# ayotoasset/AdditiveCausalExpansion

Measured on AMD Instinct MI355X. Metric: log-marg-lik+grad evals/sec at n=16384,d=20; Cholesky GF/s vs MFMA peak, higher is better.
Workload: dtype f64; 1 GPU; C2: n=16384, d=20, Matern32, ns basis B=10, fp64; one para_update (kernel assembly + SPD inverse/log-det + all P gradients + RMSE/evidence + Nadam step) per step; n=16384, p=20, B=10, kernel=Matern32, parallelism=single

## Files before the change

### additivecausalexpansion_amd/__init__.py

```python
from ._lib import AceError, Context, default_context, lib
from .native import (
    DMat, Adam_cpp, Nadam_cpp, Nesterov_cpp, coef_contract, grad_Matern_cpp, grad_SE_cpp,
    invkernel_cpp, kernmat_Matern32_cpp, kernmat_Matern32_symmetric_cpp, kernmat_SE_cpp,
    kernmat_SE_symmetric_cpp, mu_solution_cpp, ncs_basis, ncs_basis_deriv, norm_clip_cpp,
    normalize_test, normalize_train, pred_cpp, pred_marginal_cpp, robust_levels, stats_cpp,
    zero_pattern_order)
from .model import (
    BatchModel, DeviceModel, KernelClass_Matern32_R6, KernelClass_SE_R6, comm_unique_id, optAdam,
    optNadam, optNesterov, set_optimizer)
from .r6 import R6KernelMatern32, R6KernelSE
from .train import (
    AceFit, ace_train, ace_train_batch, coef_posterior, linear_spline, ns_spline, predict_ace,
    response_surface, robust_treatment, set_basis, set_initial_parameters, square_spline)
```

### additivecausalexpansion_amd/_lib.py

```python
from __future__ import annotations

import ctypes
import os
import threading

import numpy as np

_HERE = os.path.dirname(os.path.abspath(__file__))
LIB_PATH = os.environ.get("ACE_LIB_PATH") or os.path.join(_HERE, "libace_hip.so")

ACE_KERNEL_SE = 0
ACE_KERNEL_MATERN32 = 1
KIND = {"SE": ACE_KERNEL_SE, "Matern32": ACE_KERNEL_MATERN32}

_D = ctypes.POINTER(ctypes.c_double)
_I64 = ctypes.c_int64
_I32 = ctypes.POINTER(ctypes.c_int32)
_vp = ctypes.c_void_p

SIGNATURES = {
    "ace_abi_version": (ctypes.c_int, []),
    "ace_create": (ctypes.c_int, [ctypes.c_int, ctypes.POINTER(_vp)]),
    "ace_destroy": (None, [_vp]),
    "ace_last_error": (ctypes.c_char_p, [_vp]),
# ... 37 lines not shown
                                             ctypes.c_double, _vp, _vp, _vp, ctypes.c_double,
                                             ctypes.c_double, ctypes.c_double, ctypes.c_int, _D,
                                             _D, _D, _D]),
    "ace_nesterov": (ctypes.c_int, [_I64, ctypes.c_double, ctypes.c_double, _D, _D, _D]),
    "ace_nadam": (ctypes.c_int, [_I64, ctypes.c_double, ctypes.c_double, ctypes.c_double,
                                 ctypes.c_double, ctypes.c_double, _D, _D, _D, _D]),
    "ace_adam": (ctypes.c_int, [_I64, ctypes.c_double, ctypes.c_double, ctypes.c_double,
                                ctypes.c_double, ctypes.c_double, _D, _D, _D, _D]),
    "ace_norm_clip": (None, [ctypes.c_int, _I64, _D, ctypes.c_double]),
    "ace_ncs_basis": (ctypes.c_int, [_I64, _D, _I64, _D, _D, ctypes.POINTER(_I64)]),
    "ace_ncs_basis_deriv": (ctypes.c_int, [_I64, _D, _I64, _D, _D, ctypes.POINTER(_I64)]),
    "ace_normalize_train": (ctypes.c_int, [_I64, ctypes.c_int, ctypes.c_int, _D, _D, _D, _D]),
    "ace_normalize_test": (ctypes.c_int, [_I64, ctypes.c_int, ctypes.c_int, _D, _D, _D, _I64]),
    "ace_zero_pattern_order": (ctypes.c_int, [_I64, ctypes.c_int, _D, ctypes.POINTER(_I64),
                                              ctypes.POINTER(ctypes.c_uint32), _I32]),
    "ace_model_create": (ctypes.c_int, [_vp, ctypes.c_int, _I64, ctypes.c_int, ctypes.c_int,
                                        ctypes.POINTER(_vp)]),
    "ace_model_destroy": (None, [_vp]),
    "ace_model_set_data": (ctypes.c_int, [_vp, _D, _D, _D, ctypes.c_double]),
    "ace_model_para_update": (ctypes.c_int, [_vp, ctypes.c_int, _D, _D, _D, _D]),
    "ace_model_train_stats": (ctypes.c_int, [_vp, _D, _D]),
    "ace_model_get_inverse": (ctypes.c_int, [_vp, _D]),
    "ace_model_apply_inverse": (ctypes.c_int, [_vp, _I64, _D, _D]),
    "ace_model_predict": (ctypes.c_int, [_vp, _D, _I64, _D, _D, ctypes.c_double, ctypes.c_double,
                                         _D, _D, _D]),
    "ace_model_predict_marginal": (ctypes.c_int, [_vp, _D, _I64, _D, _D, _D, ctypes.c_double,
                                                  ctypes.c_double, ctypes.c_int, _D, _D, _D,
                                                  _D]),
    "ace_model_predict_marginal_groups": (ctypes.c_int, [_vp, _D, _I64, _D, _D, ctypes.c_double,
                                                         ctypes.c_double, ctypes.c_int, _I32, _D,
# ... 144 lines not shown
```

### additivecausalexpansion_amd/csrc/ace_api.cpp

```cpp
#include <hip/hip_runtime.h>
#include <hip/hip_ext.h>

#include <algorithm>
#include <chrono>
#include <cmath>
#include <cstdio>
#include <cstring>
#include <limits>
#include <string>
#include <thread>
#include <vector>

#include "../../include/ace_hip.h"

#include "ace_common.h"
#include "ace_internal.h"
#include "ace_model.h"

using namespace ace;

std::string g_create_err;

namespace {
double sync_timeout_s() {
// ... 430 lines not shown
  return v;
}
static bool asm_fill_on() {
  static const bool v = env_int("ACE_ASM_FILL", 1) != 0;
  return v;
}

struct AsmFill {
  int kind, PM, B, ZS, slots;
  PairSide ps;
  int64_t npad, naug;
  TabView tv;
  double sig;
  double *A;
  int *queue;
};

static hipError_t asm_fill(void *arg, hipStream_t st) {
  const AsmFill *f = (const AsmFill *)arg;
  return launch_assembly_persist(f->kind, f->PM, f->ps, f->npad, f->B, f->ZS, f->tv, f->sig, f->A,
                                 f->naug, st, f->queue, 0, f->slots);
}

void assemble_and_sweep(ace_ctx *ctx, SweepWork &w, const Shape &s, const PairSide &ps,
                        const TabView &tv, double sig, const double *y, int64_t n,
                        const SweepTiming *tmg, hipEvent_t *ev_asm) {
  hipStream_t st = ctx->stream;
  const int steps = (int)(w.npad / NB);
  SweepSync sy = w.sync(ctx);
  const int R = asm_persist_reserve();
  const bool persist = R > 0 && sy.side && sy.nev >= 5 * steps + 6 && pairs_use_mm(s.PM, false) &&
                       mm_lds_ok(s.PM, s.B, s.kind, false);
  ck(ctx, launch_aug_init(w.A.d(), w.naug, w.npad, n, y, st, 1, 0, w.flag.i(), 1,
                          persist ? w.aq.i() : nullptr, persist ? 2 + 64 : 0),
     "aug init");
  if (ev_asm) ck(ctx, hipEventRecord(ev_asm[0], st), "event");
  ck(ctx, launch_assembly(0, s.kind, s.PM, ps, ps, w.npad, s.B, s.ZS, tv, sig, w.A.d(), w.naug,
                          nullptr, st, nullptr, 0, 1, 1),
     "assembly (first panel)");
  if (sy.side && sy.nev >= 2 * steps + 1) {
    ck(ctx, hipEventRecord(sy.ev[2 * steps], st), "event");
    sy.ready_recorded = true;
  }
  AsmFill fill;
  if (persist && sy.ready_recorded) {
    ck(ctx, launch_assembly_persist(s.kind, s.PM, ps, w.npad, s.B, s.ZS, tv, sig, w.A.d(), w.naug,
                                    st, w.aq.i(), R),
       "assembly (persistent)");
    const int tail = asm_tail_mode();
    if (tail == 0) {
      sy.tail_after = sy.ev[5 * steps + 5];
      ck(ctx, hipEventRecord(sy.tail_after, st), "event");
    }
    sy.tail_split = tail == 2;
    const int per = asm_fill_on() ? assembly_persist_per_cu(s.kind, s.PM, s.B) : 0;
    if (per > 0) {
      fill = AsmFill{s.kind, s.PM, s.B, s.ZS, 32 * R * per, ps, w.npad, w.naug, tv, sig, w.A.d(), w.aq.i()};
      sy.fill = asm_fill;
      sy.fill_arg = &fill;
    }
  } else {
    ck(ctx, launch_assembly(0, s.kind, s.PM, ps, ps, w.npad, s.B, s.ZS, tv, sig, w.A.d(), w.naug,
                            nullptr, st, nullptr, 0, 1, 2),
       "assembly");
  }
  if (ev_asm) ck(ctx, hipEventRecord(ev_asm[1], st), "event");
  ck(ctx, run_sweep(w.bufs(), st, &sy, tmg), "sweep");
}

void build_grad_tiles(ace_ctx *ctx, int64_t n, DBuf &tiles, int64_t *ntiles, int64_t *ndiag,
                      const uint32_t *mask) {
  *ntiles = grad_ntiles(n);
// ... 52 lines not shown
    tv.ldn = m->npad;
  }
  const int ts = m->tset;
  SweepTiming tmg;
  const size_t nset = m->ev_upd.size() / 2;
  tmg.ev = m->ev_upd.data() + ts * nset;
  tmg.nev = (int)nset;
  tmg.used = &m->upd_used[ts];
  tmg.flops = m->upd_flops.data() + ts * (nset / 2);
  assemble_and_sweep(ctx, w, s, ps, tv, sig, m->y.d(), m->n, timed ? &tmg : nullptr,
                     timed ? m->ev_asm + 2 * ts : nullptr);
  ck(ctx, launch_alpha_from_aug(w.A.d(), w.naug, w.npad, m->n, theta_dev ? 0.0 : theta[1], use_mu,
                                m->alpha.d(), m->scal.d(), st, theta_dev ? theta_dev + 1 : nullptr),
     "alpha");
  if (timed) ck(ctx, hipEventRecord(m->ev_grad[2 * ts], st), "event");
  ck(ctx, launch_grad(s.kind, s.PM, ps, s.B, s.ZS, tv, w.A.d(), w.naug, -1.0, m->alpha.d(),
                      nullptr, m->gpart.d(), st, reinterpret_cast<const Tile *>(m->gtiles.p),
                      m->ngdiag >= 0 ? m->ntiles : 0, 1, m->ngdiag),
     "grad");
  if (timed) ck(ctx, hipEventRecord(m->ev_grad[2 * ts + 1], st), "event");
  const int ldg = grad_part_cols(s.PM, s.B);
  ck(ctx, launch_tile_sums(m->gpart.d(), m->ntiles, ldg, m->gwork.d(), m->gsum.d(), st),
     "tile sums");
  ck(ctx, launch_final_sums(m->y.d(), m->scal.d() + 4, m->alpha.d(), nullptr, sig, m->n,
                            w.piv.d(), w.npad, m->sums.d(), st, tv.sig, w.flag.i()),
     "final sums");
}

void model_collect_timing(ace_model *m, int ts) {
  const int nupd = m->upd_used[ts];
  const size_t nset = m->ev_upd.size() / 2;
  const hipEvent_t *ev = m->ev_upd.data() + ts * nset;
  const double *fl = m->upd_flops.data() + ts * (nset / 2);
  float ms = 0.f;
  ck(m->ctx, hipEventElapsedTime(&ms, m->ev_asm[2 * ts], m->ev_asm[2 * ts + 1]), "elapsed");
  m->t_ms[1] += ms;
  m->t_launch[1] += 1;
  ck(m->ctx, hipEventElapsedTime(&ms, m->ev_grad[2 * ts], m->ev_grad[2 * ts + 1]), "elapsed");
  m->t_ms[2] += ms;
  m->t_launch[2] += 1;
  for (int j = 0; j + 1 < nupd; j += 2) {
// ... 139 lines not shown
    alloc(ctx, m->gpart, (size_t)(m->ntiles * ldg) * sizeof(double), "alloc gpart");
    alloc(ctx, m->gwork, (size_t)tile_sums_work(ldg) * sizeof(double), "alloc tile sums");
    alloc(ctx, m->res, (size_t)(ldg + 8 + 16) * sizeof(double), "alloc results");
    m->gsum.p = m->res.d();
    m->sums.p = m->res.d() + ldg;
    m->scal.p = m->res.d() + ldg + 8;
    ck(ctx, hipMemsetAsync(m->sw.A.p, 0, m->sw.A.bytes, ctx->stream), "memset A");
    const int steps = (int)(m->npad / NB);
    m->ev_upd.assign((size_t)(4 * steps), nullptr);
    m->upd_flops.assign((size_t)(2 * steps), 0.0);
    for (auto &e : m->ev_upd) ck(ctx, hipEventCreateWithFlags(&e, ACE_TIMING_EVENT_FLAGS), "event");
    for (int j = 0; j < 4; ++j) {
      ck(ctx, hipEventCreateWithFlags(&m->ev_asm[j], ACE_TIMING_EVENT_FLAGS), "event");
      ck(ctx, hipEventCreateWithFlags(&m->ev_grad[j], ACE_TIMING_EVENT_FLAGS), "event");
    }
    sync(ctx);
  } catch (const Fail &f) {
    ace_model_destroy(m);
    return f.code;
  }
  *out = m;
  return ACE_OK;
}

void ace_model_destroy(ace_model *m) {
  if (!m) return;
  (void)hipSetDevice(m->ctx->device);
  if (m->shard) shard_destroy(m->shard);
  for (auto &e : m->ev_upd)
    if (e) (void)hipEventDestroy(e);
  for (int j = 0; j < 4; ++j) {
    if (m->ev_asm[j]) (void)hipEventDestroy(m->ev_asm[j]);
    if (m->ev_grad[j]) (void)hipEventDestroy(m->ev_grad[j]);
  }
  delete m;
}

int ace_model_set_data(ace_model *m, const double *y, const double *X, const double *Z,
                       double std_y) {
  if (!m) return ACE_ERR_ARG;
  ace_ctx *ctx = m->ctx;
  ACE_TRY
  ck(ctx, hipSetDevice(ctx->device), "hipSetDevice");
  arg(ctx, y && (m->s.p == 0 || X) && (m->s.B == 1 || Z), "null argument");
  if (m->shard) {
    shard_set_data(m->shard, y, X, Z);
    m->std_y = std_y;
    m->has_data = true;
    return ACE_OK;
  }
  const Shape &s = m->s;
  const int64_t n = m->n;
  const int zs = s.B - 1, mode = zskip_mode(n);
  m->perm.clear();
  m->has_zmask = false;
  std::vector<double> Xp, Zp, yp((size_t)m->npad, 0.0);
  std::copy(y, y + n, yp.begin());
  if (mode > 0 && zs >= 1 && zs <= 32 && pairs_use_mm(s.PM, false) &&
      mm_lds_ok(s.PM, s.B, s.kind, false) && mm_lds_ok(s.PM, s.B, s.kind, true)) {
    const uint32_t all = zs >= 32 ? 0xffffffffu : ((uint32_t)1 << zs) - 1;
    std::vector<uint32_t> bm((size_t)(m->npad / AT), all);
    std::vector<int64_t> perm((size_t)n);
    int32_t has = 0;
    arg(ctx, ace_zero_pattern_order(n, zs, Z, perm.data(), bm.data(), &has) == ACE_OK,
        "zero-pattern order");
    bool ident = true;
    for (int64_t k = 0; k < n && ident; ++k) ident = perm[(size_t)k] == k;
    if (mode == 2 && !ident) {
      Xp.resize((size_t)(n * s.p));
      Zp.resize((size_t)(n * zs));
// ... 8 lines not shown
    } else if (!ident) {
      for (int64_t k = 0; k < n / AT; ++k) {
        uint32_t w = 0;
        for (int b = 0; b < zs; ++b)
          for (int64_t j = AT * k; j < AT * (k + 1); ++j)
            if (Z[j + b * n] != 0.0) w |= (uint32_t)1 << b;
        bm[(size_t)k] = w;
      }
    }
    bool any = false;
    for (uint32_t w : bm) any = any || w != all;
    if (any) {
      alloc(ctx, m->zmask, bm.size() * sizeof(uint32_t), "alloc slice masks");
      upload_bytes(ctx, m->zmask.p, bm.data(), bm.size() * sizeof(uint32_t), "upload slice masks");
      m->has_zmask = true;
    }
    int64_t nt = 0;
    build_grad_tiles(ctx, n, m->gtiles, &nt, &m->ngdiag,
                     (any && !m->perm.empty()) ? bm.data() : nullptr);
    arg(ctx, nt == m->ntiles, "gradient tile list changed size");
  }
  upload_side(ctx, m->side, m->s, X, Z, m->n, m->npad);
  upload_bytes(ctx, m->y.p, yp.data(), yp.size() * sizeof(double), "upload y");
  m->std_y = std_y;
  sync(ctx);
  m->has_data = true;
  return ACE_OK;
  ACE_CATCH
}

// ... 303 lines not shown
```

### additivecausalexpansion_amd/csrc/ace_host.cpp

```cpp
#include <algorithm>
#include <cmath>
#include <vector>

#include "../../include/ace_hip.h"

namespace {

bool all_finite(int64_t P, const double *g) {
  for (int64_t j = 0; j < P; ++j)
    if (!std::isfinite(g[j])) return false;
  return true;
}

}

extern "C" {

int ace_nesterov(int64_t P, double learn_rate, double momentum, double *nu, const double *grad,
                 double *para) {
  const bool ok = all_finite(P, grad);
  for (int64_t j = 0; j < P; ++j) {
    nu[j] = momentum * nu[j] + learn_rate * grad[j];
    para[j] = para[j] + nu[j];
  }
// ... 242 lines not shown
  const bool mask = ZS <= 32 && blockmask != nullptr;
  if (has_mask) *has_mask = mask ? 1 : 0;
  if (!mask) return ACE_OK;
  const uint32_t all = ZS >= 32 ? 0xffffffffu : ((uint32_t)1 << ZS) - 1;
  const int64_t nblk = (n + 63) / 64;
  for (int64_t k = 0; k < nblk; ++k) {
    uint32_t m = 0;
    if (64 * (k + 1) > n) m = all;
    else
      for (int64_t j = 64 * k; j < 64 * (k + 1); ++j) m |= (uint32_t)pat[(size_t)perm[j] * W];
    blockmask[k] = m;
  }
  return ACE_OK;
}

int ace_coef_contract(int64_t nx, int B, int64_t nz, const double *mean, const double *cov,
                      const double *W, double offset, double scale, double shift, double noise,
                      double *map, double *ci, double *var) {
  if (nx < 1 || nz < 1 || B < 1 || !mean || !cov || !W || !map || !ci || !var) return ACE_ERR_ARG;
  const int64_t N = nx * nz;
  std::vector<double> wj((size_t)B);
  for (int64_t j = 0; j < nz; ++j) {
    for (int b = 0; b < B; ++b) wj[(size_t)b] = W[j + nz * b];
    for (int64_t c = 0; c < nx; ++c) {
      double a = 0.0, q = 0.0;
      for (int b = 0; b < B; ++b) a += wj[(size_t)b] * mean[c + nx * b];
      for (int b2 = 0; b2 < B; ++b2) {
        double t = 0.0;
        for (int b = 0; b < B; ++b) t += wj[(size_t)b] * cov[c + nx * (b + (int64_t)B * b2)];
        q += t * wj[(size_t)b2];
// ... 15 lines not shown
```

### additivecausalexpansion_amd/csrc/ace_internal.h

```cpp
#pragma once
#include <functional>
#include <vector>
#include <hip/hip_runtime.h>
#include <stdint.h>
#include <stdlib.h>

namespace ace {

inline int env_int(const char *name, int dflt) {
  const char *e = getenv(name);
  return e ? atoi(e) : dflt;
}
inline bool env_set(const char *name) { return getenv(name) != nullptr; }

#ifndef ACE_NB
#define ACE_NB 256
#endif
constexpr int NB = ACE_NB;
constexpr int SUB = 64;
constexpr int UT = 128;
constexpr int AUG = 128;
constexpr int AT = 64;
constexpr int PMAX = 64;
constexpr int BMAX = 32;
// ... 30 lines not shown
hipError_t launch_assembly(int mode, int kind, int PM, PairSide rows,
                           PairSide cols, int64_t npad, int B, int ZS,
                           TabView tab, double sig, double *out, int64_t ld,
                           double *cube, hipStream_t st, const Tile *tiles = nullptr,
                           int64_t ntiles = 0, int G = 1, int part = 0, int b0 = 0,
                           int b1 = -1);
hipError_t launch_kdiag(int kind, PairSide S, int ZS, TabView tab, int b0, int b1, double *out,
                        hipStream_t st);

hipError_t launch_assembly_mm(int kind, int PM, PairSide S, int64_t npad, int B, int ZS,
                              TabView tab, double sig, double *out, int64_t ld,
                              double *kcopy, hipStream_t st, const Tile *tiles,
                              int64_t ntiles, int G, int part = 0);
hipError_t launch_assembly_persist(int kind, int PM, PairSide S, int64_t npad, int B, int ZS,
                                   TabView tab, double sig, double *out, int64_t ld,
                                   hipStream_t st, int *queue, int reserve, int fill = 0);
int assembly_persist_per_cu(int kind, int PM, int B);
bool pairs_use_mm(int PM, bool grad);
bool mm_lds_ok(int PM, int B, int kind, bool grad);
bool cross_mm_lds_ok(int PM, int B, int kind);
hipError_t launch_cross_mm(int kind, int PM, PairSide R, PairSide C, int B, int ZS, TabView tab,
                           int b0, int b1, double *out, int64_t ld, hipStream_t st);
hipError_t launch_cross_slices_mm(int kind, int PM, PairSide R, PairSide C, int B, int ZS,
                                  TabView tab, double *out, int64_t ld, hipStream_t st);
int group_sums_parts(int64_t n);
hipError_t launch_group_sums(int kind, int PM, PairSide S, int B, int ZS, TabView tab, int b0,
                             int b1, const int *label, int G, double *part, double *R,
                             hipStream_t st);
hipError_t launch_grad_mm(int kind, int PM, PairSide S, int B, int ZS, TabView tab,
                          const double *A, int64_t ld, double sA, const double *alpha,
                          double *gpart, hipStream_t st, const Tile *tiles, int64_t ntiles, int G,
                          int64_t ndiag);

__host__ __device__ constexpr int grad_part_cols(int PM, int B) { return B * (PM + 1) + 1; }
hipError_t launch_grad(int kind, int PM, PairSide side, int B, int ZS,
                       TabView tab, const double *A, int64_t ld, double sA,
                       const double *alpha, const double *cube, double *gpart, hipStream_t st,
                       const Tile *tiles = nullptr, int64_t ntiles = 0, int G = 1,
                       int64_t ndiag = -1);
int64_t grad_ntiles(int64_t n);
int grad_order_block();
hipError_t launch_tile_sums(const double *part, int64_t ntiles, int ncols, double *work,
                            double *out, hipStream_t st);
int64_t tile_sums_work(int ncols);

constexpr int64_t SW_DOUBLES = 2 * (int64_t)SUB * SUB + 3 * (int64_t)NB * SUB;
struct SweepBufs {
  double *A;
  int64_t ld;
  int64_t npad;
  double *P[8];
  double *W[8];
  int Z = 2;
  double *SW;
// ... 181 lines not shown
```

### additivecausalexpansion_amd/csrc/ace_model.h

```cpp
#pragma once
#include <functional>

#include "ace_common.h"
#include "ace_internal.h"

struct SweepWork {
  DBuf A, Ps[8], Ws[8], SW, S0, S1, piv, flag, order, xtiles, gorder, htiles;
  int Z = 2;
  DBuf gtiles;
  DBuf aq;
  DBuf bq;
  int breserve = 0;
  int64_t bq_npad = -1;
  int bq_Z = 0;
  DBuf gpart, gwork, gsum;
  DBuf norms;
  int64_t ngtiles = 0, ngdiag = -2;
  std::vector<int64_t> xoff, hoff;
  int64_t glen = 0;
  std::vector<hipEvent_t> ev;
  int64_t n = 0, npad = 0, naug = 0, norder = 0;
  SweepWork() = default;
  SweepWork(const SweepWork &) = delete;
  ~SweepWork() {
    for (auto &e : ev) (void)hipEventDestroy(e);
// ... 1 lines not shown
  void ensure(ace_ctx *ctx, int64_t n_) {
    n = n_;
    npad = round_up(n, NB);
    naug = npad + AUG;
    alloc(ctx, A, (size_t)(naug * naug) * sizeof(double), "alloc A");
    for (int j = 0; j < 2; ++j) {
      alloc(ctx, Ps[j], (size_t)(naug * NB) * sizeof(double), "alloc panel");
      alloc(ctx, Ws[j], (size_t)(naug * NB) * sizeof(double), "alloc panel");
    }
    alloc(ctx, SW, (size_t)SW_DOUBLES * sizeof(double), "alloc SW");
    alloc(ctx, S0, (size_t)(SUB * NB) * sizeof(double), "alloc S");
    alloc(ctx, S1, (size_t)(SUB * NB) * sizeof(double), "alloc S");
    alloc(ctx, piv, (size_t)npad * sizeof(double), "alloc piv");
    alloc(ctx, flag, 16, "alloc flag");
    alloc(ctx, aq, (2 + 64) * sizeof(int), "alloc assembly queue");
    norder = 0;
    if (const int S = update_order_block(); S > 0) {
      const std::vector<Tile> t = xcd_update_order(own_tiles(naug / UT, UT, 1, 0), S);
      alloc(ctx, order, t.size() * sizeof(Tile), "alloc tile order");
      upload_bytes(ctx, order.p, t.data(), t.size() * sizeof(Tile), "upload tile order");
      norder = (int64_t)t.size();
    }
    const int steps = (int)(npad / NB);
    glen = 0;
    hoff.clear();
    if (pair_steps() && steps >= 2) {
      Z = sweep_group_n(naug);
      for (int j = 2; j < 2 * Z; ++j) {
        alloc(ctx, Ps[j], (size_t)(naug * NB) * sizeof(double), "alloc panel");
        alloc(ctx, Ws[j], (size_t)(naug * NB) * sizeof(double), "alloc panel");
// ... 83 lines not shown
  tv.ldn = np;
  return tv;
}

struct ace_model {
  ace_ctx *ctx = nullptr;
  Shape s{};
  int64_t n = 0, npad = 0, naug = 0, ntiles = 0, ntr = 0;
  double std_y = 1.0;
  bool has_data = false;
  bool has_inverse = false;
  SideBufs side;
  std::vector<int64_t> perm;
  DBuf zmask;
  bool has_zmask = false;
  PairSide train_side() const {
    PairSide ps = side.view(n);
    if (has_zmask) ps.mask = static_cast<const uint32_t *>(zmask.p);
    return ps;
  }
  DBuf y, tab, alpha, gpart, gwork;
  DBuf res;
  DView gsum, sums, scal;
  DBuf norms;
  DBuf gtiles;
  int64_t ngdiag = -1;
  PinnedBuf hio;
  SweepWork sw;
  SweepWork sw2;
  bool prof = false;
  hipEvent_t ev_asm[4] = {}, ev_grad[4] = {};
  std::vector<hipEvent_t> ev_upd;
  std::vector<double> upd_flops;
  int upd_used[2] = {0, 0};
  int tset = 0, pend = -1;
  double t_ms[6] = {0, 0, 0, 0, 0, 0};
  int64_t t_launch[6] = {0, 0, 0, 0, 0, 0};
  double t_work[6] = {0, 0, 0, 0, 0, 0};
  ShardModel *shard = nullptr;
};


void assemble_and_sweep(ace_ctx *ctx, SweepWork &w, const Shape &s, const PairSide &ps,
                        const TabView &tv, double sig, const double *y, int64_t n,
                        const SweepTiming *tmg, hipEvent_t *ev_asm);
void build_grad_tiles(ace_ctx *ctx, int64_t n, DBuf &tiles, int64_t *ntiles, int64_t *ndiag,
// ... 20 lines not shown
```

### additivecausalexpansion_amd/csrc/ace_pairs.hip

```cpp
#include <algorithm>
#include <cstdlib>

#include "ace_internal.h"

namespace ace {

#define SQRT3 1.7320508075688772

__device__ __forceinline__ double sgn(double x) {
  return (double)((0.0 < x) - (x < 0.0));
}

template <int KIND, bool CROSS>
__device__ __forceinline__ double kval(int b, double r2, double lam, double zlo,
                                       double zhi, double lzlo, double lzhi) {
  if (KIND == 0) {
    if (b == 0) return exp(lam - r2);
    if (zlo == 0.0 || zhi == 0.0) return 0.0;
    return (sgn(zlo) * sgn(zhi)) * exp(((lam - r2) + lzlo) + lzhi);
  } else {
    const double t = sqrt(r2);
    const double e = (1.0 + SQRT3 * t) * exp(lam - SQRT3 * t);
    if (b == 0) return e;
    if (zlo == 0.0) return 0.0;
// ... 618 lines not shown
    hipLaunchKernelGGL((k_grad2<PM, 1>), grid, blk, 0, st, S, B, ZS, tab, A, ld, sA, alpha,
                       gpart, ldg, tiles, G);
  }
#undef ACE_G
  return hipGetLastError();
}

int grad_order_block() {
  static const int v = std::max(0, env_int("ACE_GRAD_ORDER", 4));
  return v;
}

hipError_t launch_grad(int kind, int PM, PairSide S, int B, int ZS, TabView tab,
                       const double *A, int64_t ld, double sA, const double *alpha,
                       const double *cube, double *gpart, hipStream_t st,
                       const Tile *tiles, int64_t ntiles, int G, int64_t ndiag) {
  const bool valu_ok = PM <= 48;
  if ((!cube || !valu_ok) && (pairs_use_mm(PM, true) || !valu_ok) && mm_lds_ok(PM, B, kind, true))
    return launch_grad_mm(kind, PM, S, B, ZS, tab, A, ld, sA, alpha, gpart, st, tiles, ntiles,
                          G, ndiag);
  if (!valu_ok) return hipErrorInvalidValue;
  switch (PM) {
#define ACE_CASE(P) \
  case P:           \
    return grad_pm<P>(kind, S, B, ZS, tab, A, ld, sA, alpha, cube, gpart, st, tiles, ntiles, G);
    ACE_CASE(4) ACE_CASE(8) ACE_CASE(12) ACE_CASE(16) ACE_CASE(20) ACE_CASE(24)
    ACE_CASE(32) ACE_CASE(48)
#undef ACE_CASE
    default: return hipErrorInvalidValue;
  }
}

}
```

### additivecausalexpansion_amd/csrc/ace_pairs_mm.hip

```cpp
#include <map>
#include <mutex>
#include <tuple>
#include <type_traits>

#include "ace_internal.h"
#include "ace_wgtime.h"

namespace ace {

typedef double d4 __attribute__((ext_vector_type(4)));

#ifndef ACE_MM_PG
#define ACE_MM_PG 2
#endif
#ifndef ACE_MM_GRAD_WPE
#define ACE_MM_GRAD_WPE 4
#endif
#ifndef ACE_MM_QG
#define ACE_MM_QG 4
#endif
#ifndef ACE_MM_QG2
#define ACE_MM_QG2 1
#endif
#ifndef ACE_GRAD_TAIL4
// ... 366 lines not shown
    s = fma(v * v, w[i], s);
  }
  norms[e] = s;
}

hipError_t launch_slice_norms(const double *X, int PM, int64_t np, int B, int NS,
                              const double *wk, const double *wlast, double *norms,
                              hipStream_t st) {
  const int64_t tot = (int64_t)NS * np;
  if (tot == 0) return hipSuccess;
  hipLaunchKernelGGL(k_slice_norms, dim3((unsigned)((tot + 255) / 256)), dim3(256), 0, st, X, PM,
                     np, B, NS, wk, wlast, norms);
  return hipGetLastError();
}

static int asm_first_cols(int nt) {
  const int jb = sweep_group_n((int64_t)nt * AT + AUG) * NB / AT;
  return jb < nt ? jb : nt;
}

constexpr int ASM_NT = 256;
template <int PM, int KIND, bool LOWER = false>
__device__ __forceinline__ void asm_mm_tile(double *lds, PairSide S, int B, int ZS, const TabView &tab,
                                            double sg, double *__restrict__ out, int64_t ld,
                                            double *__restrict__ kcopy, int64_t I, int64_t J,
                                            int G) {
  if (G > 1) {
    const int64_t coff = lcol(J * AT, G) - J * AT;
    out += coff * ld;
    if (kcopy) kcopy += coff * ld;
  }
// ... 226 lines not shown
    cross_slice_pairs<PM, KIND>(kf, XJ, W, Nr, Nc, Zc, LZc, E, xr, tab, b, zr, lzr, rl, lr, lk);
  }
  if (!rok) return;
#pragma unroll
  for (int cb = 0; cb < 4; ++cb)
#pragma unroll
    for (int v = 0; v < 4; ++v) {
      const int64_t c = C0 + 16 * cb + lk + 4 * v;
      if (c < C.n) out[r + c * ld] = kf[cb][v];
    }
}

template <int PM, int KIND>
__global__ __launch_bounds__(ASM_NT, PM <= 24 ? 4 : PM <= 32 ? 3 : 2) void k_asm_mm_q(
    PairSide S, int B, int ZS, TabView tab, double sig, double *__restrict__ out, int64_t ld,
    int *__restrict__ queue, int64_t nblk, int JB, int reserve) {
  extern __shared__ __attribute__((aligned(16))) double lds[];
  __shared__ int next;
  if (reserve > 0) {
    if (threadIdx.x == 0) {
      const unsigned hw = __builtin_amdgcn_s_getreg((31 << 11) | 4);
      const unsigned xcc = __builtin_amdgcn_s_getreg((31 << 11) | 20) & 7;
      const unsigned se = (hw >> 13) & 3;
      const int key = (int)((hw >> 8) & 0xff) + 1;
      int mine = 0;
      for (int r = 0; r < reserve && !mine; ++r) {
        const int old = atomicCAS(queue + 2 + 2 * (4 * xcc + se) + r, 0, key);
        mine = old == 0 || old == key;
      }
      next = mine ? (atomicAdd(queue + 1, 1) < (int)gridDim.x * reserve / 4) : 0;
    }
    __syncthreads();
    if (next) return;
    __syncthreads();
  }
  const double sg = tab.sig ? *tab.sig : sig;
  for (;;) {
    if (threadIdx.x == 0) next = atomicAdd(queue, 1);
    __syncthreads();
    const int64_t idx = next;
    __syncthreads();
    if (idx >= nblk) break;
    int64_t I, J;
    tile_of(nullptr, idx, I, J);
    asm_mm_tile<PM, KIND, true>(lds, S, B, ZS, tab, sg, out, ld, nullptr, I + JB + 1, J + JB, 1);
  }
}

__device__ __forceinline__ double rcp_nr_mm(double f) {
  const double q = __builtin_amdgcn_rcp(f);
  const double e = fma(-f, q, 1.0);
  return fma(q, e, q);
}

template <int CTRL>
__device__ __forceinline__ double dpp64(double v) {
  const unsigned long long u = __double_as_longlong(v);
  const int lo = __builtin_amdgcn_mov_dpp((int)(unsigned)u, CTRL, 0xf, 0xf, false);
  const int hi = __builtin_amdgcn_mov_dpp((int)(unsigned)(u >> 32), CTRL, 0xf, 0xf, false);
  return __longlong_as_double((long long)(((unsigned long long)(unsigned)hi << 32) | (unsigned)lo));
// ... 413 lines not shown
static hipError_t grad_mm_launch_ps(PairSide S, int B, int ZS, TabView tab, const double *A,
                                    int64_t ld, double sA, const double *alpha, double *gpart,
                                    hipStream_t st, const Tile *tiles, int64_t nblk, int G,
                                    size_t lds, int64_t t0) {
  constexpr int CB = grad_cb(PM, KIND);
  constexpr int NT = 64 * 4 * (4 / CB);
  if (nblk == 0) return hipSuccess;
  return launch_lds(k_grad_mm<PM, KIND, CB, PS, DG>, dim3((unsigned)nblk), dim3(NT), lds, st, S, B,
                    ZS, tab, A, ld, sA, alpha, gpart, grad_part_cols(PM, B), tiles, G, t0);
}

template <int PM, int KIND, bool PS>
static hipError_t grad_mm_launch_dg(PairSide S, int B, int ZS, TabView tab, const double *A,
                                    int64_t ld, double sA, const double *alpha, double *gpart,
                                    hipStream_t st, const Tile *tiles, int64_t nslot,
                                    int64_t ndiag, int G, size_t lds) {
  if (tiles && ndiag < 0)
    return grad_mm_launch_ps<PM, KIND, PS, true>(S, B, ZS, tab, A, ld, sA, alpha, gpart, st, tiles,
                                                 nslot, G, lds, 0);
  const int64_t nd = tiles ? ndiag : (S.n + AT - 1) / AT;
  hipError_t e = grad_mm_launch_ps<PM, KIND, PS, false>(S, B, ZS, tab, A, ld, sA, alpha, gpart, st,
                                                        tiles, nslot - nd, G, lds, nd);
  if (e != hipSuccess) return e;
  return grad_mm_launch_ps<PM, KIND, PS, true>(S, B, ZS, tab, A, ld, sA, alpha, gpart, st, tiles,
                                               nd, G, lds, 0);
}

template <int PM, int KIND>
static hipError_t grad_mm_launch(PairSide S, int B, int ZS, TabView tab, const double *A,
                                 int64_t ld, double sA, const double *alpha, double *gpart,
                                 hipStream_t st, const Tile *tiles, int64_t nslot, int64_t ndiag,
                                 int G) {
  constexpr int CB = grad_cb(PM, KIND);
  constexpr int NT = 64 * 4 * (4 / CB);
  const MmLayout o = mm_layout(PM, B, KIND, true, NT / 64);
  const size_t lds = (size_t)o.total * sizeof(double);
  return o.red_slices == B
             ? grad_mm_launch_dg<PM, KIND, true>(S, B, ZS, tab, A, ld, sA, alpha, gpart, st, tiles,
                                                 nslot, ndiag, G, lds)
             : grad_mm_launch_dg<PM, KIND, false>(S, B, ZS, tab, A, ld, sA, alpha, gpart, st,
                                                  tiles, nslot, ndiag, G, lds);
}

bool mm_lds_ok(int PM, int B, int kind, bool grad) {
  const int nwave = grad ? 4 * (4 / grad_cb(PM, kind)) : 4;
  return (int64_t)mm_layout(PM, B, kind == 0 ? 0 : 1, grad, nwave).total *
             (int64_t)sizeof(double) <=
         160 * 1024;
}

hipError_t launch_grad_mm(int kind, int PM, PairSide S, int B, int ZS, TabView tab,
                          const double *A, int64_t ld, double sA, const double *alpha,
                          double *gpart, hipStream_t st, const Tile *tiles, int64_t ntiles, int G,
                          int64_t ndiag) {
  return with_pm(PM, [&](auto pm) {
    const int64_t nt = (S.n + AT - 1) / AT;
    const int64_t nslot = tiles ? ntiles : nt * (nt + 1) / 2;
    if (nslot == 0) return hipSuccess;
    return with_kind(kind, [&](auto kd) {
      return grad_mm_launch<decltype(pm)::value, decltype(kd)::value>(
          S, B, ZS, tab, A, ld, sA, alpha, gpart, st, tiles, nslot, ndiag, G);
    });
  });
}

template <int PM, int KIND>
static hipError_t asm_mm_launch(PairSide S, int64_t npad, int B, int ZS, TabView tab, double sig,
                                double *out, int64_t ld, double *kcopy, hipStream_t st,
                                const Tile *tiles, int64_t ntiles, int G, int part) {
  const int64_t nt = npad / AT, JB = asm_first_cols((int)nt);
  if (tiles) part = 0;
  const int64_t nblk = tiles ? ntiles
                       : part == 1 ? JB * nt - JB * (JB - 1) / 2
                       : part == 2 ? (nt - JB) * (nt - JB + 1) / 2
                       : part == 3 ? nt - JB
                                   : nt * (nt + 1) / 2;
  if (nblk == 0) return hipSuccess;
  const size_t lds = (size_t)mm_layout(PM, B, KIND, false).total * sizeof(double);
  return launch_lds(k_asm_mm<PM, KIND>, dim3((unsigned)nblk), dim3(ASM_NT), lds, st, S, B, ZS, tab,
                    sig, out, ld, kcopy, tiles, G, part, nt, JB);
}

template <int PM, int KIND>
static hipError_t asm_mm_persist_launch(PairSide S, int64_t npad, int B, int ZS, TabView tab,
                                        double sig, double *out, int64_t ld, hipStream_t st,
                                        int *queue, int reserve, int slots, bool fill) {
  const int64_t nt = npad / AT, JB = asm_first_cols((int)nt);
  const int64_t nblk = (nt - JB) * (nt - JB - 1) / 2;
  if (nt - JB <= 0) return hipSuccess;
  const size_t lds = (size_t)mm_layout(PM, B, KIND, false).total * sizeof(double);
  const hipError_t e = fill ? hipSuccess
                            : asm_mm_launch<PM, KIND>(S, npad, B, ZS, tab, sig, out, ld, nullptr,
                                                      st, nullptr, 0, 1, 3);
  if (e != hipSuccess || nblk == 0) return e;
  if (fill) reserve = 0;
  return launch_lds(k_asm_mm_q<PM, KIND>, dim3((unsigned)slots), dim3(ASM_NT), lds, st, S, B, ZS,
                    tab, sig, out, ld, queue, nblk, JB, reserve);
}

template <int PM>
static int asm_mm_slots(int kind, int B) {
  int dev = 0, ncu = 0, per = 0;
  if (hipGetDevice(&dev) != hipSuccess) return 0;
  static std::mutex mu;
  static std::map<std::tuple<int, int, int>, int> cache;
  const auto key = std::make_tuple(dev, kind, B);
  {
    std::lock_guard<std::mutex> g(mu);
    const auto it = cache.find(key);
    if (it != cache.end()) return it->second;
  }
  if (hipDeviceGetAttribute(&ncu, hipDeviceAttributeMultiprocessorCount, dev) != hipSuccess)
// ... 23 lines not shown
    return hipSuccess;
  });
  return per;
}

#ifdef ACE_DIAG_WGTIME
}
extern "C" long long ace_diag_wgtime_pairs(void *dst, long long cap, int reset) {
  return ace::wgt_read(dst, cap, reset);
}
namespace ace {
#endif

hipError_t launch_assembly_persist(int kind, int PM, PairSide S, int64_t npad, int B, int ZS,
                                   TabView tab, double sig, double *out, int64_t ld,
                                   hipStream_t st, int *queue, int reserve, int fill) {
  return with_pm(PM, [&](auto pm) {
    constexpr int P = decltype(pm)::value;
    const int slots = fill > 0 ? fill : asm_mm_slots<P>(kind, B);
    if (slots <= 0) return hipErrorInvalidValue;
    return with_kind(kind, [&](auto kd) {
      return asm_mm_persist_launch<P, decltype(kd)::value>(S, npad, B, ZS, tab, sig, out, ld, st,
                                                           queue, reserve, slots, fill > 0);
    });
  });
}

static size_t cross_mm_lds(int PM, int B, int kind) {
  return (size_t)(mm_layout(PM, B, kind == 0 ? 0 : 1, false).total + 64 * xj_pitch(PM)) *
         sizeof(double);
}
bool cross_mm_lds_ok(int PM, int B, int kind) { return cross_mm_lds(PM, B, kind) <= 160 * 1024; }

hipError_t launch_cross_mm(int kind, int PM, PairSide R, PairSide C, int B, int ZS, TabView tab,
                           int b0, int b1, double *out, int64_t ld, hipStream_t st) {
  return with_pm(PM, [&](auto pm) {
    constexpr int P = decltype(pm)::value;
    if (R.n <= 0 || C.n <= 0 || b1 <= b0) return hipSuccess;
// ... 265 lines not shown
```

### additivecausalexpansion_amd/native.py

```python
from __future__ import annotations

import ctypes

import numpy as np

from ._lib import KIND, AceError, check, default_context, fmat, lib, ptr


def _ctx(ctx):
    return (ctx or default_context()).handle


class DMat:

    def __init__(self, handle, ctx):
        self.handle, self.ctx = handle, ctx
        r, c, sl = ctypes.c_int64(), ctypes.c_int64(), ctypes.c_int64()
        check(lib().ace_dmat_dims(handle, ctypes.byref(r), ctypes.byref(c), ctypes.byref(sl)))
        self.shape = (r.value, c.value) if sl.value == 1 else (r.value, c.value, sl.value)

    @classmethod
    def upload(cls, a, ctx=None):
        a = np.asarray(a, dtype=np.float64)
        dims = a.shape + (1,) * (3 - a.ndim)
# ... 351 lines not shown
def zero_pattern_order(Z):
    Zf = fmat(Z)
    if Zf.ndim != 2 or Zf.shape[0] < 1:
        raise AceError("Z must be n x ZS with n >= 1")
    n, ZS = Zf.shape
    perm = np.empty(n, dtype=np.int64)
    mask = np.zeros((n + 63) // 64, dtype=np.uint32)
    has = np.zeros(1, dtype=np.int32)
    check(lib().ace_zero_pattern_order(n, ZS, ptr(Zf) if ZS else None,
                                       perm.ctypes.data_as(ctypes.POINTER(ctypes.c_int64)),
                                       mask.ctypes.data_as(ctypes.POINTER(ctypes.c_uint32)),
                                       has.ctypes.data_as(ctypes.POINTER(ctypes.c_int32))))
    return perm, (mask if has[0] else None)


def coef_contract(mean, cov, W, offset=0.0, scale=1.0, shift=0.0, noise=0.0):
    mf = fmat(mean)
    if mf.ndim != 2:
        raise AceError("mean must be nx x B")
    nx, B = mf.shape
    cf = np.asfortranarray(np.asarray(cov, dtype=np.float64).reshape((nx, B, B), order="F"))
    Wf = np.asfortranarray(np.asarray(W, dtype=np.float64).reshape((-1, B), order="F"))
    nz = Wf.shape[0]
    mp = np.empty((nx, nz), order="F")
    var = np.empty((nx, nz), order="F")
    ci = np.empty((nx, nz, 2), order="F")
    check(lib().ace_coef_contract(nx, B, nz, ptr(mf), cf.ctypes.data_as(ctypes.POINTER(ctypes.c_double)),
                                  ptr(Wf), float(offset), float(scale), float(shift), float(noise),
                                  ptr(mp), ci.ctypes.data_as(ctypes.POINTER(ctypes.c_double)),
                                  ptr(var)))
# ... 2 lines not shown
```

### include/ace_hip.h

```cpp
#ifndef ACE_HIP_H
#define ACE_HIP_H

#include <stdint.h>

#ifdef __cplusplus
extern "C" {
#endif

#define ACE_ABI_VERSION 1

enum ace_kernel_kind { ACE_KERNEL_SE = 0, ACE_KERNEL_MATERN32 = 1 };

enum ace_status {
  ACE_OK = 0,
  ACE_ERR_ARG = 1,
  ACE_ERR_HIP = 2,
  ACE_ERR_OOM = 3,
  ACE_ERR_UNSUPPORTED = 4,
  ACE_ERR_NONFINITE = 5,
  ACE_ERR_INTERRUPTED = 6,
  ACE_ERR_TIMEOUT = 7
};

typedef struct ace_ctx ace_ctx;
// ... 87 lines not shown

void ace_norm_clip(int flag, int64_t P, double *grads, double max_length);

int ace_ncs_basis(int64_t n, const double *x, int64_t nknots,
                  const double *knots, double *design, int64_t *ncols);
int ace_ncs_basis_deriv(int64_t n, const double *x, int64_t nknots,
                        const double *knots, double *design, int64_t *ncols);

int ace_normalize_train(int64_t n, int px, int pz, double *y, double *X,
                        double *Z, double *moments);
int ace_normalize_test(int64_t n, int px, int pz, double *X, double *Z,
                       const double *moments, int64_t moment_rows);

int ace_zero_pattern_order(int64_t n, int ZS, const double *Z, int64_t *perm,
                           uint32_t *blockmask, int32_t *has_mask);

int ace_model_create(ace_ctx *ctx, int kind, int64_t n, int p, int B,
                     ace_model **out);
void ace_model_destroy(ace_model *m);
int ace_model_set_data(ace_model *m, const double *y, const double *X,
                       const double *Z, double std_y);
int ace_model_para_update(ace_model *m, int iter, double *theta, double *grad,
                          double *stats, double *mu_post);
int ace_model_train_stats(ace_model *m, const double *theta, double *stats);
int ace_model_get_inverse(ace_model *m, double *inv);
int ace_model_apply_inverse(ace_model *m, int64_t k, const double *V, double *out);

int ace_model_predict(ace_model *m, const double *theta, int64_t nx, const double *X2,
                      const double *Z2, double mean_y, double std_y, double *map, double *ci,
                      double *var);
// ... 82 lines not shown
```

Measured before the change: 14.25 evals/s.

## Order assembly tiles by slice-mask cost and overlap grad tail on side streams

The persistent assembly kernel now reads its tile coordinates from a precomputed tile list instead of deriving them from the queue index. When a zero-pattern mask exists, that list is sorted so tiles with the most active slices come first, which should reduce load imbalance at the end of the queue. Separately, the diagonal-tile grad launch and the final-sums kernel now run on two side streams joined with events, so they can overlap with the main grad and tile-sum work. The cost is extra event traffic and a small uploaded tile buffer, and the stream split adds ordering risks.

```diff
diff --git a/additivecausalexpansion_amd/__init__.py b/additivecausalexpansion_amd/__init__.py
--- a/additivecausalexpansion_amd/__init__.py
+++ b/additivecausalexpansion_amd/__init__.py
@@ -1,7 +1,7 @@
 from ._lib import AceError, Context, default_context, lib
 from .native import (
-    DMat, Adam_cpp, Nadam_cpp, Nesterov_cpp, coef_contract, grad_Matern_cpp, grad_SE_cpp,
-    invkernel_cpp, kernmat_Matern32_cpp, kernmat_Matern32_symmetric_cpp, kernmat_SE_cpp,
+    DMat, Adam_cpp, Nadam_cpp, Nesterov_cpp, asm_tile_order, coef_contract, grad_Matern_cpp,
+    grad_SE_cpp, invkernel_cpp, kernmat_Matern32_cpp, kernmat_Matern32_symmetric_cpp, kernmat_SE_cpp,
     kernmat_SE_symmetric_cpp, mu_solution_cpp, ncs_basis, ncs_basis_deriv, norm_clip_cpp,
     normalize_test, normalize_train, pred_cpp, pred_marginal_cpp, robust_levels, stats_cpp,
     zero_pattern_order)
diff --git a/additivecausalexpansion_amd/_lib.py b/additivecausalexpansion_amd/_lib.py
--- a/additivecausalexpansion_amd/_lib.py
+++ b/additivecausalexpansion_amd/_lib.py
@@ -75,6 +75,7 @@
     "ace_normalize_test": (ctypes.c_int, [_I64, ctypes.c_int, ctypes.c_int, _D, _D, _D, _I64]),
     "ace_zero_pattern_order": (ctypes.c_int, [_I64, ctypes.c_int, _D, ctypes.POINTER(_I64),
                                               ctypes.POINTER(ctypes.c_uint32), _I32]),
+    "ace_asm_tile_order": (ctypes.c_int, [_I64, _I64, ctypes.POINTER(ctypes.c_uint32), _I32]),
     "ace_model_create": (ctypes.c_int, [_vp, ctypes.c_int, _I64, ctypes.c_int, ctypes.c_int,
                                         ctypes.POINTER(_vp)]),
     "ace_model_destroy": (None, [_vp]),
diff --git a/additivecausalexpansion_amd/csrc/ace_api.cpp b/additivecausalexpansion_amd/csrc/ace_api.cpp
--- a/additivecausalexpansion_amd/csrc/ace_api.cpp
+++ b/additivecausalexpansion_amd/csrc/ace_api.cpp
@@ -468,12 +468,14 @@
   double sig;
   double *A;
   int *queue;
+  const Tile *tiles;
+  int64_t ntiles;
 };
 
 static hipError_t asm_fill(void *arg, hipStream_t st) {
   const AsmFill *f = (const AsmFill *)arg;
   return launch_assembly_persist(f->kind, f->PM, f->ps, f->npad, f->B, f->ZS, f->tv, f->sig, f->A,
-                                 f->naug, st, f->queue, 0, f->slots);
+                                 f->naug, st, f->queue, 0, f->tiles, f->ntiles, f->slots);
 }
 
 void assemble_and_sweep(ace_ctx *ctx, SweepWork &w, const Shape &s, const PairSide &ps,
@@ -499,7 +501,7 @@
   AsmFill fill;
   if (persist && sy.ready_recorded) {
     ck(ctx, launch_assembly_persist(s.kind, s.PM, ps, w.npad, s.B, s.ZS, tv, sig, w.A.d(), w.naug,
-                                    st, w.aq.i(), R),
+                                    st, w.aq.i(), R, w.asm_tiles(), w.natiles),
        "assembly (persistent)");
     const int tail = asm_tail_mode();
     if (tail == 0) {
@@ -509,7 +511,8 @@
     sy.tail_split = tail == 2;
     const int per = asm_fill_on() ? assembly_persist_per_cu(s.kind, s.PM, s.B) : 0;
     if (per > 0) {
-      fill = AsmFill{s.kind, s.PM, s.B, s.ZS, 32 * R * per, ps, w.npad, w.naug, tv, sig, w.A.d(), w.aq.i()};
+      fill = AsmFill{s.kind, s.PM, s.B, s.ZS, 32 * R * per, ps, w.npad, w.naug, tv, sig, w.A.d(), w.aq.i(),
+                     w.asm_tiles(), w.natiles};
       sy.fill = asm_fill;
       sy.fill_arg = &fill;
     }
@@ -592,17 +595,25 @@
                                 m->alpha.d(), m->scal.d(), st, theta_dev ? theta_dev + 1 : nullptr),
      "alpha");
   if (timed) ck(ctx, hipEventRecord(m->ev_grad[2 * ts], st), "event");
+  hipEvent_t *const evt = m->ev_tail;
+  ck(ctx, hipEventRecord(evt[0], st), "event");
+  ck(ctx, hipStreamWaitEvent(ctx->side, evt[0], 0), "wait");
+  ck(ctx, hipStreamWaitEvent(ctx->side2, evt[0], 0), "wait");
   ck(ctx, launch_grad(s.kind, s.PM, ps, s.B, s.ZS, tv, w.A.d(), w.naug, -1.0, m->alpha.d(),
                       nullptr, m->gpart.d(), st, reinterpret_cast<const Tile *>(m->gtiles.p),
-                      m->ngdiag >= 0 ? m->ntiles : 0, 1, m->ngdiag),
+                      m->ngdiag >= 0 ? m->ntiles : 0, 1, m->ngdiag, ctx->side),
      "grad");
+  ck(ctx, hipEventRecord(evt[1], ctx->side), "event");
+  ck(ctx, launch_final_sums(m->y.d(), m->scal.d() + 4, m->alpha.d(), nullptr, sig, m->n,
+                            w.piv.d(), w.npad, m->sums.d(), ctx->side2, tv.sig, w.flag.i()),
+     "final sums");
+  ck(ctx, hipEventRecord(evt[2], ctx->side2), "event");
+  ck(ctx, hipStreamWaitEvent(st, evt[1], 0), "wait");
   if (timed) ck(ctx, hipEventRecord(m->ev_grad[2 * ts + 1], st), "event");
   const int ldg = grad_part_cols(s.PM, s.B);
   ck(ctx, launch_tile_sums(m->gpart.d(), m->ntiles, ldg, m->gwork.d(), m->gsum.d(), st),
      "tile sums");
-  ck(ctx, launch_final_sums(m->y.d(), m->scal.d() + 4, m->alpha.d(), nullptr, sig, m->n,
-                            w.piv.d(), w.npad, m->sums.d(), st, tv.sig, w.flag.i()),
-     "final sums");
+  ck(ctx, hipStreamWaitEvent(st, evt[2], 0), "wait");
 }
 
 void model_collect_timing(ace_model *m, int ts) {
@@ -772,6 +783,7 @@
       ck(ctx, hipEventCreateWithFlags(&m->ev_asm[j], ACE_TIMING_EVENT_FLAGS), "event");
       ck(ctx, hipEventCreateWithFlags(&m->ev_grad[j], ACE_TIMING_EVENT_FLAGS), "event");
     }
+    for (auto &e : m->ev_tail) ck(ctx, hipEventCreateWithFlags(&e, ACE_SYNC_EVENT_FLAGS), "event");
     sync(ctx);
   } catch (const Fail &f) {
     ace_model_destroy(m);
@@ -791,6 +803,8 @@
     if (m->ev_asm[j]) (void)hipEventDestroy(m->ev_asm[j]);
     if (m->ev_grad[j]) (void)hipEventDestroy(m->ev_grad[j]);
   }
+  for (auto &e : m->ev_tail)
+    if (e) (void)hipEventDestroy(e);
   delete m;
 }
 
@@ -812,6 +826,7 @@
   const int zs = s.B - 1, mode = zskip_mode(n);
   m->perm.clear();
   m->has_zmask = false;
+  m->sw.atiles_ov = m->sw2.atiles_ov = nullptr;
   std::vector<double> Xp, Zp, yp((size_t)m->npad, 0.0);
   std::copy(y, y + n, yp.begin());
   if (mode > 0 && zs >= 1 && zs <= 32 && pairs_use_mm(s.PM, false) &&
@@ -850,6 +865,9 @@
       alloc(ctx, m->zmask, bm.size() * sizeof(uint32_t), "alloc slice masks");
       upload_bytes(ctx, m->zmask.p, bm.data(), bm.size() * sizeof(uint32_t), "upload slice masks");
       m->has_zmask = true;
+      arg(ctx, upload_asm_tiles(ctx, m->atiles, m->npad, bm.data()) == m->sw.natiles,
+          "assembly tile list changed size");
+      m->sw.atiles_ov = m->sw2.atiles_ov = reinterpret_cast<const Tile *>(m->atiles.p);
     }
     int64_t nt = 0;
     build_grad_tiles(ctx, n, m->gtiles, &nt, &m->ngdiag,
diff --git a/additivecausalexpansion_amd/csrc/ace_host.cpp b/additivecausalexpansion_amd/csrc/ace_host.cpp
--- a/additivecausalexpansion_amd/csrc/ace_host.cpp
+++ b/additivecausalexpansion_amd/csrc/ace_host.cpp
@@ -280,6 +280,29 @@
   return ACE_OK;
 }
 
+int ace_asm_tile_order(int64_t nt, int64_t jb, const uint32_t *mask, int32_t *tiles) {
+  if (nt < 0 || jb < 0 || nt > INT32_MAX) return ACE_ERR_ARG;
+  const int64_t m = nt - jb;
+  if (m < 2) return ACE_OK;
+  if (!tiles) return ACE_ERR_ARG;
+  struct T {
+    int32_t I, J;
+  };
+  std::vector<T> lst;
+  lst.reserve((size_t)(m * (m - 1) / 2));
+  for (int64_t I = jb + 1; I < nt; ++I)
+    for (int64_t J = jb; J < I; ++J) lst.push_back(T{(int32_t)I, (int32_t)J});
+  if (mask)
+    std::stable_sort(lst.begin(), lst.end(), [mask](const T &a, const T &b) {
+      return __builtin_popcount(mask[a.I] & mask[a.J]) > __builtin_popcount(mask[b.I] & mask[b.J]);
+    });
+  for (size_t k = 0; k < lst.size(); ++k) {
+    tiles[2 * k] = lst[k].I;
+    tiles[2 * k + 1] = lst[k].J;
+  }
+  return ACE_OK;
+}
+
 int ace_coef_contract(int64_t nx, int B, int64_t nz, const double *mean, const double *cov,
                       const double *W, double offset, double scale, double shift, double noise,
                       double *map, double *ci, double *var) {
diff --git a/additivecausalexpansion_amd/csrc/ace_internal.h b/additivecausalexpansion_amd/csrc/ace_internal.h
--- a/additivecausalexpansion_amd/csrc/ace_internal.h
+++ b/additivecausalexpansion_amd/csrc/ace_internal.h
@@ -68,7 +68,9 @@
                               int64_t ntiles, int G, int part = 0);
 hipError_t launch_assembly_persist(int kind, int PM, PairSide S, int64_t npad, int B, int ZS,
                                    TabView tab, double sig, double *out, int64_t ld,
-                                   hipStream_t st, int *queue, int reserve, int fill = 0);
+                                   hipStream_t st, int *queue, int reserve, const Tile *tiles,
+                                   int64_t ntiles, int fill = 0);
+int asm_first_cols(int nt);
 int assembly_persist_per_cu(int kind, int PM, int B);
 bool pairs_use_mm(int PM, bool grad);
 bool mm_lds_ok(int PM, int B, int kind, bool grad);
@@ -84,14 +86,14 @@
 hipError_t launch_grad_mm(int kind, int PM, PairSide S, int B, int ZS, TabView tab,
                           const double *A, int64_t ld, double sA, const double *alpha,
                           double *gpart, hipStream_t st, const Tile *tiles, int64_t ntiles, int G,
-                          int64_t ndiag);
+                          int64_t ndiag, hipStream_t st_diag = nullptr);
 
 __host__ __device__ constexpr int grad_part_cols(int PM, int B) { return B * (PM + 1) + 1; }
 hipError_t launch_grad(int kind, int PM, PairSide side, int B, int ZS,
                        TabView tab, const double *A, int64_t ld, double sA,
                        const double *alpha, const double *cube, double *gpart, hipStream_t st,
                        const Tile *tiles = nullptr, int64_t ntiles = 0, int G = 1,
-                       int64_t ndiag = -1);
+                       int64_t ndiag = -1, hipStream_t st_diag = nullptr);
 int64_t grad_ntiles(int64_t n);
 int grad_order_block();
 hipError_t launch_tile_sums(const double *part, int64_t ntiles, int ncols, double *work,
diff --git a/additivecausalexpansion_amd/csrc/ace_model.h b/additivecausalexpansion_amd/csrc/ace_model.h
--- a/additivecausalexpansion_amd/csrc/ace_model.h
+++ b/additivecausalexpansion_amd/csrc/ace_model.h
@@ -3,12 +3,29 @@
 
 #include "ace_common.h"
 #include "ace_internal.h"
+
+inline int64_t upload_asm_tiles(ace_ctx *ctx, DBuf &buf, int64_t npad, const uint32_t *mask) {
+  const int64_t nt = npad / AT, m = nt - asm_first_cols((int)nt);
+  const int64_t cnt = m >= 2 ? m * (m - 1) / 2 : 0;
+  static_assert(sizeof(Tile) == 2 * sizeof(int32_t), "Tile is two ints");
+  std::vector<int32_t> t((size_t)(2 * cnt));
+  arg(ctx, ace_asm_tile_order(nt, nt - m, mask, t.data()) == ACE_OK, "assembly tile order");
+  alloc(ctx, buf, std::max<size_t>(t.size(), 2) * sizeof(int32_t), "alloc assembly tiles");
+  if (cnt > 0) upload_bytes(ctx, buf.p, t.data(), t.size() * sizeof(int32_t), "upload assembly tiles");
+  return cnt;
+}
 
 struct SweepWork {
   DBuf A, Ps[8], Ws[8], SW, S0, S1, piv, flag, order, xtiles, gorder, htiles;
   int Z = 2;
   DBuf gtiles;
   DBuf aq;
+  DBuf atiles;
+  int64_t natiles = 0, atiles_npad = -1;
+  const Tile *atiles_ov = nullptr;
+  const Tile *asm_tiles() const {
+    return atiles_ov ? atiles_ov : reinterpret_cast<const Tile *>(atiles.p);
+  }
   DBuf bq;
   int breserve = 0;
   int64_t bq_npad = -1;
@@ -40,6 +57,10 @@
     alloc(ctx, piv, (size_t)npad * sizeof(double), "alloc piv");
     alloc(ctx, flag, 16, "alloc flag");
     alloc(ctx, aq, (2 + 64) * sizeof(int), "alloc assembly queue");
+    if (atiles_npad != npad) {
+      natiles = upload_asm_tiles(ctx, atiles, npad, nullptr);
+      atiles_npad = npad;
+    }
     norder = 0;
     if (const int S = update_order_block(); S > 0) {
       const std::vector<Tile> t = xcd_update_order(own_tiles(naug / UT, UT, 1, 0), S);
@@ -153,6 +174,7 @@
   std::vector<int64_t> perm;
   DBuf zmask;
   bool has_zmask = false;
+  DBuf atiles;
   PairSide train_side() const {
     PairSide ps = side.view(n);
     if (has_zmask) ps.mask = static_cast<const uint32_t *>(zmask.p);
@@ -169,6 +191,7 @@
   SweepWork sw2;
   bool prof = false;
   hipEvent_t ev_asm[4] = {}, ev_grad[4] = {};
+  hipEvent_t ev_tail[3] = {};
   std::vector<hipEvent_t> ev_upd;
   std::vector<double> upd_flops;
   int upd_used[2] = {0, 0};
diff --git a/additivecausalexpansion_amd/csrc/ace_pairs.hip b/additivecausalexpansion_amd/csrc/ace_pairs.hip
--- a/additivecausalexpansion_amd/csrc/ace_pairs.hip
+++ b/additivecausalexpansion_amd/csrc/ace_pairs.hip
@@ -656,11 +656,12 @@
 hipError_t launch_grad(int kind, int PM, PairSide S, int B, int ZS, TabView tab,
                        const double *A, int64_t ld, double sA, const double *alpha,
                        const double *cube, double *gpart, hipStream_t st,
-                       const Tile *tiles, int64_t ntiles, int G, int64_t ndiag) {
+                       const Tile *tiles, int64_t ntiles, int G, int64_t ndiag,
+                       hipStream_t st_diag) {
   const bool valu_ok = PM <= 48;
   if ((!cube || !valu_ok) && (pairs_use_mm(PM, true) || !valu_ok) && mm_lds_ok(PM, B, kind, true))
     return launch_grad_mm(kind, PM, S, B, ZS, tab, A, ld, sA, alpha, gpart, st, tiles, ntiles,
-                          G, ndiag);
+                          G, ndiag, st_diag);
   if (!valu_ok) return hipErrorInvalidValue;
   switch (PM) {
 #define ACE_CASE(P) \
diff --git a/additivecausalexpansion_amd/csrc/ace_pairs_mm.hip b/additivecausalexpansion_amd/csrc/ace_pairs_mm.hip
--- a/additivecausalexpansion_amd/csrc/ace_pairs_mm.hip
+++ b/additivecausalexpansion_amd/csrc/ace_pairs_mm.hip
@@ -404,7 +404,7 @@
   return hipGetLastError();
 }
 
-static int asm_first_cols(int nt) {
+int asm_first_cols(int nt) {
   const int jb = sweep_group_n((int64_t)nt * AT + AUG) * NB / AT;
   return jb < nt ? jb : nt;
 }
@@ -661,7 +661,7 @@
 template <int PM, int KIND>
 __global__ __launch_bounds__(ASM_NT, PM <= 24 ? 4 : PM <= 32 ? 3 : 2) void k_asm_mm_q(
     PairSide S, int B, int ZS, TabView tab, double sig, double *__restrict__ out, int64_t ld,
-    int *__restrict__ queue, int64_t nblk, int JB, int reserve) {
+    int *__restrict__ queue, int64_t nblk, const Tile *__restrict__ tiles, int reserve) {
   extern __shared__ __attribute__((aligned(16))) double lds[];
   __shared__ int next;
   if (reserve > 0) {
@@ -688,9 +688,8 @@
     const int64_t idx = next;
     __syncthreads();
     if (idx >= nblk) break;
-    int64_t I, J;
-    tile_of(nullptr, idx, I, J);
-    asm_mm_tile<PM, KIND, true>(lds, S, B, ZS, tab, sg, out, ld, nullptr, I + JB + 1, J + JB, 1);
+    const Tile t = tiles[idx];
+    asm_mm_tile<PM, KIND, true>(lds, S, B, ZS, tab, sg, out, ld, nullptr, t.I, t.J, 1);
   }
 }
 
@@ -1134,7 +1133,7 @@
 static hipError_t grad_mm_launch_dg(PairSide S, int B, int ZS, TabView tab, const double *A,
                                     int64_t ld, double sA, const double *alpha, double *gpart,
                                     hipStream_t st, const Tile *tiles, int64_t nslot,
-                                    int64_t ndiag, int G, size_t lds) {
+                                    int64_t ndiag, int G, size_t lds, hipStream_t st_diag) {
   if (tiles && ndiag < 0)
     return grad_mm_launch_ps<PM, KIND, PS, true>(S, B, ZS, tab, A, ld, sA, alpha, gpart, st, tiles,
                                                  nslot, G, lds, 0);
@@ -1142,24 +1141,24 @@
   hipError_t e = grad_mm_launch_ps<PM, KIND, PS, false>(S, B, ZS, tab, A, ld, sA, alpha, gpart, st,
                                                         tiles, nslot - nd, G, lds, nd);
   if (e != hipSuccess) return e;
-  return grad_mm_launch_ps<PM, KIND, PS, true>(S, B, ZS, tab, A, ld, sA, alpha, gpart, st, tiles,
-                                               nd, G, lds, 0);
+  return grad_mm_launch_ps<PM, KIND, PS, true>(S, B, ZS, tab, A, ld, sA, alpha, gpart,
+                                               st_diag ? st_diag : st, tiles, nd, G, lds, 0);
 }
 
 template <int PM, int KIND>
 static hipError_t grad_mm_launch(PairSide S, int B, int ZS, TabView tab, const double *A,
                                  int64_t ld, double sA, const double *alpha, double *gpart,
                                  hipStream_t st, const Tile *tiles, int64_t nslot, int64_t ndiag,
-                                 int G) {
+                                 int G, hipStream_t st_diag) {
   constexpr int CB = grad_cb(PM, KIND);
   constexpr int NT = 64 * 4 * (4 / CB);
   const MmLayout o = mm_layout(PM, B, KIND, true, NT / 64);
   const size_t lds = (size_t)o.total * sizeof(double);
   return o.red_slices == B
              ? grad_mm_launch_dg<PM, KIND, true>(S, B, ZS, tab, A, ld, sA, alpha, gpart, st, tiles,
-                                                 nslot, ndiag, G, lds)
+                                                 nslot, ndiag, G, lds, st_diag)
              : grad_mm_launch_dg<PM, KIND, false>(S, B, ZS, tab, A, ld, sA, alpha, gpart, st,
-                                                  tiles, nslot, ndiag, G, lds);
+                                                  tiles, nslot, ndiag, G, lds, st_diag);
 }
 
 bool mm_lds_ok(int PM, int B, int kind, bool grad) {
@@ -1172,14 +1171,14 @@
 hipError_t launch_grad_mm(int kind, int PM, PairSide S, int B, int ZS, TabView tab,
                           const double *A, int64_t ld, double sA, const double *alpha,
                           double *gpart, hipStream_t st, const Tile *tiles, int64_t ntiles, int G,
-                          int64_t ndiag) {
+                          int64_t ndiag, hipStream_t st_diag) {
   return with_pm(PM, [&](auto pm) {
     const int64_t nt = (S.n + AT - 1) / AT;
     const int64_t nslot = tiles ? ntiles : nt * (nt + 1) / 2;
     if (nslot == 0) return hipSuccess;
     return with_kind(kind, [&](auto kd) {
       return grad_mm_launch<decltype(pm)::value, decltype(kd)::value>(
-          S, B, ZS, tab, A, ld, sA, alpha, gpart, st, tiles, nslot, ndiag, G);
+          S, B, ZS, tab, A, ld, sA, alpha, gpart, st, tiles, nslot, ndiag, G, st_diag);
     });
   });
 }
@@ -1204,10 +1203,12 @@
 template <int PM, int KIND>
 static hipError_t asm_mm_persist_launch(PairSide S, int64_t npad, int B, int ZS, TabView tab,
                                         double sig, double *out, int64_t ld, hipStream_t st,
-                                        int *queue, int reserve, int slots, bool fill) {
+                                        int *queue, int reserve, int slots, bool fill,
+                                        const Tile *tiles, int64_t ntiles) {
   const int64_t nt = npad / AT, JB = asm_first_cols((int)nt);
   const int64_t nblk = (nt - JB) * (nt - JB - 1) / 2;
   if (nt - JB <= 0) return hipSuccess;
+  if (ntiles != nblk || (nblk > 0 && !tiles)) return hipErrorInvalidValue;
   const size_t lds = (size_t)mm_layout(PM, B, KIND, false).total * sizeof(double);
   const hipError_t e = fill ? hipSuccess
                             : asm_mm_launch<PM, KIND>(S, npad, B, ZS, tab, sig, out, ld, nullptr,
@@ -1215,7 +1216,7 @@
   if (e != hipSuccess || nblk == 0) return e;
   if (fill) reserve = 0;
   return launch_lds(k_asm_mm_q<PM, KIND>, dim3((unsigned)slots), dim3(ASM_NT), lds, st, S, B, ZS,
-                    tab, sig, out, ld, queue, nblk, JB, reserve);
+                    tab, sig, out, ld, queue, nblk, tiles, reserve);
 }
 
 template <int PM>
@@ -1269,14 +1270,16 @@
 
 hipError_t launch_assembly_persist(int kind, int PM, PairSide S, int64_t npad, int B, int ZS,
                                    TabView tab, double sig, double *out, int64_t ld,
-                                   hipStream_t st, int *queue, int reserve, int fill) {
+                                   hipStream_t st, int *queue, int reserve, const Tile *tiles,
+                                   int64_t ntiles, int fill) {
   return with_pm(PM, [&](auto pm) {
     constexpr int P = decltype(pm)::value;
     const int slots = fill > 0 ? fill : asm_mm_slots<P>(kind, B);
     if (slots <= 0) return hipErrorInvalidValue;
     return with_kind(kind, [&](auto kd) {
       return asm_mm_persist_launch<P, decltype(kd)::value>(S, npad, B, ZS, tab, sig, out, ld, st,
-                                                           queue, reserve, slots, fill > 0);
+                                                           queue, reserve, slots, fill > 0, tiles,
+                                                           ntiles);
     });
   });
 }
diff --git a/additivecausalexpansion_amd/native.py b/additivecausalexpansion_amd/native.py
--- a/additivecausalexpansion_amd/native.py
+++ b/additivecausalexpansion_amd/native.py
@@ -389,6 +389,23 @@
     return perm, (mask if has[0] else None)
 
 
+def asm_tile_order(nt, jb, mask=None):
+    nt, jb = int(nt), int(jb)
+    m = max(nt - jb, 0)
+    tiles = np.zeros((m * (m - 1) // 2, 2), dtype=np.int32)
+    mk = None
+    if mask is not None:
+        mk = np.ascontiguousarray(mask, dtype=np.uint32)
+        if mk.size != nt:
+            raise AceError("mask must hold nt words")
+    check(lib().ace_asm_tile_order(nt, jb,
+                                   mk.ctypes.data_as(ctypes.POINTER(ctypes.c_uint32))
+                                   if mk is not None else None,
+                                   tiles.ctypes.data_as(ctypes.POINTER(ctypes.c_int32))
+                                   if tiles.size else None))
+    return tiles
+
+
 def coef_contract(mean, cov, W, offset=0.0, scale=1.0, shift=0.0, noise=0.0):
     mf = fmat(mean)
     if mf.ndim != 2:
diff --git a/include/ace_hip.h b/include/ace_hip.h
--- a/include/ace_hip.h
+++ b/include/ace_hip.h
@@ -125,6 +125,9 @@
 
 int ace_zero_pattern_order(int64_t n, int ZS, const double *Z, int64_t *perm,
                            uint32_t *blockmask, int32_t *has_mask);
+
+int ace_asm_tile_order(int64_t nt, int64_t jb, const uint32_t *blockmask,
+                       int32_t *tiles);
 
 int ace_model_create(ace_ctx *ctx, int kind, int64_t n, int p, int B,
                      ace_model **out);
```

New measurement: 14.23 evals/s (median of 3 runs). Within noise of the previous version (-0.1%).
